# binli123/dsmil-wsi

Measured on AMD Instinct MI355X. Metric: bags/sec aggregated (10kx512), higher is better.
Workload: dtype f32; 1 GPU; DSMIL aggregator forward (FCLayer+BClassifier), c16 weights C=1, 64 bags x 10000 x 512 fp32 per GPU per pass, HBM-resident; bags_per_pass_per_gpu=64, rows=10000, feats=512, classes=1, tile_rows=128, parallelism=bag-sharded x1, streams=3, distinct_batches=3, logits_form=1, device_cus=256, persistent_grid=256

## Files before the change

dsmil-wsi_amd/csrc/agg_f2.h:

```cpp
#pragma once
#include "agg_hs.h"

namespace {

typedef _Float16 f16x8 __attribute__((ext_vector_type(8)));
typedef _Float16 f16x2 __attribute__((ext_vector_type(2)));
union F2Frag {
    unsigned u[4];
    f16x8 v;
    f32x4 f;
    f16x2 h[4];
};

constexpr int F2_BM = 64;
constexpr int F2_THREADS = 512;
constexpr int F2_MAXSTEPS = 32;
constexpr int F2_XP_F4 = F2_MAXSTEPS * 2 * 2 * F2_BM;
constexpr int F2_HP_F4 = 2 * 4 * 2 * F2_BM;
constexpr int F2_SCR = 2720;
constexpr int F2_LDS_BYTES = (F2_XP_F4 + F2_HP_F4) * 16 + F2_SCR * 4;
constexpr int F2_CHUNK_F4 = 4 * 2 * 64;
constexpr int F2_WRD = 8;
constexpr int F2_WLA = 6;
constexpr int F2_STAGGER = 0;
// ... 262 lines not shown
        const float* src = row_src(cur, sc, sinv);
        hand_over(0, true, cur, sinv);
        sQall[tid - 256] = load_q(cur);

#pragma unroll
        for (int c = 0; c < NK1; ++c) {
            ring[c][0] = *(const DSMIL_GLOBAL f32x4*)(src + 32 * c);
            ring[c][1] = *(const DSMIL_GLOBAL f32x4*)(src + 32 * c + 4);
        }
        int nitem = item + stride;
        F2Tile nxt = cur;
        bool have_next = f2_fetch(a, tiles_per_bag, n_items, stride, nitem, nxt);
        const float* nsrc = have_next ? row_src(nxt, nsc, nsinv) : src;
        __syncthreads();
        int par = 0;
        f32x4* dst0 = sXp + (long long)((o >> 1) * 4 + (o & 1)) * F2_BM + 16 * j + rr;
        while (have) {
            STAMP(0);
            const float qn = load_q(nxt);
            hand_over(par ^ 1, have_next, nxt, nsinv);
            auto refill = [&](int k) {
                if constexpr ((ABL & 2) == 0) {
                    if constexpr ((ABL & 64) != 0) {
                        ring[k][0] = __builtin_nontemporal_load((const DSMIL_GLOBAL f32x4*)(nsrc + 32 * k));
                        ring[k][1] = __builtin_nontemporal_load((const DSMIL_GLOBAL f32x4*)(nsrc + 32 * k + 4));
                    } else {
                        ring[k][0] = *(const DSMIL_GLOBAL f32x4*)(nsrc + 32 * k);
                        ring[k][1] = *(const DSMIL_GLOBAL f32x4*)(nsrc + 32 * k + 4);
                    }
                }
            };
#pragma unroll
            for (int c = 0; c < NK1; ++c) {
                if constexpr ((ABL & 16) == 0) {
                    F2Frag f[2];
                    split2h_scaled(ring[c][0], ring[c][1], sc, f);
                    f32x4* dst = dst0 + (long long)c * (8 * F2_BM);
                    dst[0] = f[0].f;
                    dst[2 * F2_BM] = f[1].f;
                }
                if constexpr ((ABL & 2) == 0) {
                    if constexpr ((ABL & 256) != 0) { if (c % 2 == 1) refill(c / 2); }
                    else if (c < NK1 / 2) refill(c);
                }
                if (c < NK1 / 2 || c % 4 == 3) __syncthreads();
                if (c == 0) STAMP(1);
                if (c == 3) STAMP(2);
                if (c == 7) STAMP(3);
                if (c == 11) STAMP(4);
                if (c == NK1 - 1) STAMP(5);
            }
            sQall[(par ^ 1) * 256 + (tid - 256)] = qn;
            int nnitem = nitem + stride;
            F2Tile nn = nxt;
            bool have_nn = false;
            float nnsc = nsc, nnsinv = nsinv;
            const float* nnsrc = nsrc;
            auto look_record = [&]() { have_nn = have_next && f2_fetch(a, tiles_per_bag, n_items, stride, nnitem, nn); };
            auto look_rows = [&]() { if (have_nn) nnsrc = row_src(nn, nnsc, nnsinv); };
            auto refill_q = [&](int q) {
                if constexpr (NK1 % 8 == 0) {
#pragma unroll
                    for (int k = NK1 / 2 + q * (NK1 / 8); k < NK1 / 2 + (q + 1) * (NK1 / 8); ++k) refill(k);
                } else if (q == 0) {
#pragma unroll
                    for (int k = NK1 / 2; k < NK1; ++k) refill(k);
                }
            };
            if (a.nonlinear) {
                refill_q(0); __syncthreads();
                refill_q(1); __syncthreads();
                look_record();
                refill_q(2); __syncthreads();
                refill_q(3); __syncthreads();
                look_rows();
            } else {
                refill_q(0); refill_q(1); refill_q(2); refill_q(3);
                look_record(); look_rows();
            }
            asm volatile("" : "+v"(nnsc), "+v"(nnsinv), "+v"(nnsrc));
            STAMP(6);
            f2_tail<ABL>(a, cur, noq, sXp, sS, sPw, sQall + par * 256, sInvAll + par * F2_BM, NKS);
            STAMP(7);
            STAMP_OUT(cur);
            item = nitem; cur = nxt; have = have_next; src = nsrc; sc = nsc;
            nitem = nnitem; nxt = nn; have_next = have_nn; nsrc = nnsrc; nsc = nnsc; nsinv = nnsinv;
            par ^= 1;
        }
        return;
    }

    const char* wbase = reinterpret_cast<const char*>(wimg + (2 * wave) * 64);
    const unsigned loff = (unsigned)lane * 16u;
    F2Frag wr[F2_WRD][2];
    auto load_w = [&](auto slot_, int s) {
        constexpr int R = decltype(slot_)::value;
        if constexpr ((ABL & 1) != 0) return;
        int sw = s < nst ? s : s - nst;
        asm volatile("" : "+s"(sw));
        const char* p = wbase + (size_t)sw * (F2_CHUNK_F4 * 16);
        wr[R][0].f = *(const DSMIL_GLOBAL f32x4*)(p + loff);
        wr[R][1].f = *(const DSMIL_GLOBAL f32x4*)(p + 1024 + loff);
    };
    auto read_x = [&](int s, F2Frag (&fb)[2][2]) {
        const f32x4* p = sXp + (long long)(s * 4 + hi) * F2_BM + l31;
#pragma unroll
        for (int g = 0; g < 2; ++g) {
            fb[g][0].f = p[32 * g];
            fb[g][1].f = p[2 * F2_BM + 32 * g];
        }
    };
    auto read_h = [&](int st, F2Frag (&fb)[2][2]) {
        const f32x4* p = sHp + (long long)((st & 3) * 2 + hi) * F2_BM + l31;
#pragma unroll
        for (int g = 0; g < 2; ++g) {
            fb[g][0].f = p[32 * g];
            fb[g][1].f = p[8 * F2_BM + 32 * g];
        }
    };
    auto mfma6 = [&](f32x16 (&acc)[2], const F2Frag (&w)[2], const F2Frag (&x)[2][2]) {
        if constexpr ((ABL & 4) != 0) {
            acc[0][0] += w[0].f[0] + w[1].f[0] + x[0][0].f[0] + x[0][1].f[0];
            acc[1][0] += x[1][0].f[0] + x[1][1].f[0];
            return;
        }
#pragma unroll
        for (int g = 0; g < 2; ++g) acc[g] = __builtin_amdgcn_mfma_f32_32x32x16_f16(w[1].v, x[g][0].v, acc[g], 0, 0, 0);
#pragma unroll
        for (int g = 0; g < 2; ++g) acc[g] = __builtin_amdgcn_mfma_f32_32x32x16_f16(w[0].v, x[g][1].v, acc[g], 0, 0, 0);
#pragma unroll
        for (int g = 0; g < 2; ++g) acc[g] = __builtin_amdgcn_mfma_f32_32x32x16_f16(w[0].v, x[g][0].v, acc[g], 0, 0, 0);
    };
    using F_ = std::false_type;
    using T_ = std::true_type;
    static_assert(F2_WRD == 8, "step groups below");
    constexpr int WLA = (ABL & 128) ? 7 : F2_WLA;
    load_w(std::integral_constant<int, 0>{}, 0);
    load_w(std::integral_constant<int, 1>{}, 1);
    load_w(std::integral_constant<int, 2>{}, 2);
    load_w(std::integral_constant<int, 3>{}, 3);
    load_w(std::integral_constant<int, 4>{}, 4);
    load_w(std::integral_constant<int, 5>{}, 5);
    if constexpr (WLA == 7) load_w(std::integral_constant<int, 6>{}, 6);
    const float ia1 = trailer[0], ia2 = trailer[1];
    __syncthreads();
    int par = 0;
    while (true) {
        const int* ctl = reinterpret_cast<const int*>(sCtl + par * 8);
        auto ctl64 = [&](int i) {
            const unsigned lo = (unsigned)__builtin_amdgcn_readfirstlane(ctl[2 * i]), hi_ = (unsigned)__builtin_amdgcn_readfirstlane(ctl[2 * i + 1]);
            return (long long)(((unsigned long long)hi_ << 32) | lo);
        };
        if (__builtin_amdgcn_readfirstlane(ctl[0]) == 0) break;
        cur.bag = (int)ctl64(1); cur.off0 = ctl64(2); cur.Nb = ctl64(3); cur.row0 = ctl64(4); cur.slot = ctl64(5);
        const float* sInv = sInvAll + par * F2_BM;
        STAMP(0);
        f32x16 Hw[2], Qw[2];
#pragma unroll
        for (int g = 0; g < 2; ++g)
#pragma unroll
            for (int r = 0; r < 16; ++r) Hw[g][r] = 0.f;
        __syncthreads();
        STAMP(1);
        F2Frag xb[2][2];
        read_x(0, xb);
#pragma unroll
        for (int s = 0; s < NKS; ++s) {
            const bool pre = s + 1 < NKS;
            if ((s & 1) && pre && f2_group_first<NK1>((s + 1) / 2)) __syncthreads();
            __builtin_amdgcn_sched_barrier(0);
            switch ((s + WLA) % 8) {
                case 0: load_w(std::integral_constant<int, 0>{}, s + WLA); break;
                case 1: load_w(std::integral_constant<int, 1>{}, s + WLA); break;
                case 2: load_w(std::integral_constant<int, 2>{}, s + WLA); break;
                case 3: load_w(std::integral_constant<int, 3>{}, s + WLA); break;
                case 4: load_w(std::integral_constant<int, 4>{}, s + WLA); break;
                case 5: load_w(std::integral_constant<int, 5>{}, s + WLA); break;
                case 6: load_w(std::integral_constant<int, 6>{}, s + WLA); break;
                default: load_w(std::integral_constant<int, 7>{}, s + WLA); break;
            }
            __builtin_amdgcn_sched_barrier(0);
            F2Frag xn[2][2];
            if (pre) read_x(s + 1, xn);
            mfma6(Hw, wr[s % 8], xb);
            if (pre) {
#pragma unroll
                for (int g = 0; g < 2; ++g)
#pragma unroll
                    for (int p = 0; p < 2; ++p) xb[g][p] = xn[g][p];
            }
            __builtin_amdgcn_sched_barrier(0);
            if (s == 7) STAMP(2);
            if (s == 15) STAMP(3);
            if (s == 23) STAMP(4);
        }
        STAMP(5);
        const float inv_sc[2] = {sInv[l31], sInv[32 + l31]};
#pragma unroll
        for (int q = 0; q < 4; ++q) {
            const f32x4 bq = *reinterpret_cast<const f32x4*>(sBias + 32 * wave + 8 * q + 4 * hi);
#pragma unroll
            for (int g = 0; g < 2; ++g) {
                const float iv = ia1 * inv_sc[g];
#pragma unroll
                for (int e = 0; e < 4; ++e) {
                    const float v = fmaf(Hw[g][4 * q + e], iv, bq[e]);
                    Hw[g][4 * q + e] = a.nonlinear ? fmaxf(v, 0.f) : v;
                }
            }
        }
        if (!a.nonlinear) {
#pragma unroll
            for (int g = 0; g < 2; ++g) Qw[g] = Hw[g];
        } else {
#pragma unroll
            for (int g = 0; g < 2; ++g) {
                float m = 0.f;
#pragma unroll
                for (int r = 0; r < 16; ++r) m = fmaxf(m, Hw[g][r]);
                m = fmaxf(m, __shfl_xor(m, 32, 64));
                if (hi == 0) sMax[wave * F2_BM + 32 * g + l31] = m;
            }
            __syncthreads();
            STAMP(6);
            float hsc[2], hinv[2];
#pragma unroll
            for (int g = 0; g < 2; ++g) {
                const int r = 32 * g + l31;
                const float m = fmaxf(fmaxf(sMax[r], sMax[F2_BM + r]), fmaxf(sMax[2 * F2_BM + r], sMax[3 * F2_BM + r]));
                hsc[g] = f2_scale(m, hinv[g]);
            }
            auto publish_h = [&]() {
#pragma unroll
                for (int g = 0; g < 2; ++g)
#pragma unroll
                    for (int sx = 0; sx < 2; ++sx) {
                        const f32x4 h0 = {Hw[g][8 * sx], Hw[g][8 * sx + 1], Hw[g][8 * sx + 2], Hw[g][8 * sx + 3]};
                        const f32x4 h1 = {Hw[g][8 * sx + 4], Hw[g][8 * sx + 5], Hw[g][8 * sx + 6], Hw[g][8 * sx + 7]};
                        F2Frag f[2];
                        split2h_scaled(h0, h1, hsc[g], f);
                        f32x4* dst = sHp + (long long)((2 * (wave & 1) + sx) * 2 + hi) * F2_BM + 32 * g + l31;
                        dst[0] = f[0].f;
                        dst[8 * F2_BM] = f[1].f;
                    }
            };
#pragma unroll
            for (int g = 0; g < 2; ++g)
#pragma unroll
                for (int r = 0; r < 16; ++r) Qw[g][r] = 0.f;
            auto step2 = [&](auto ri, auto pre_, int st) {
                constexpr int RI = decltype(ri)::value;
                constexpr bool PRE = decltype(pre_)::value;
                __builtin_amdgcn_sched_barrier(0);
                load_w(std::integral_constant<int, (RI + WLA) % F2_WRD>{}, NKS + st + WLA);
                __builtin_amdgcn_sched_barrier(0);
                F2Frag xn[2][2];
                if constexpr (PRE) read_h(st + 1, xn);
                mfma6(Qw, wr[RI], xb);
                if constexpr (PRE) {
#pragma unroll
                    for (int g = 0; g < 2; ++g)
#pragma unroll
                        for (int p = 0; p < 2; ++p) xb[g][p] = xn[g][p];
                }
                __builtin_amdgcn_sched_barrier(0);
            };
            if (wave < 2) publish_h();
            __syncthreads();
            STAMP(7);
            read_h(0, xb);
            step2(std::integral_constant<int, 0>{}, T_{}, 0);
            step2(std::integral_constant<int, 1>{}, T_{}, 1);
            step2(std::integral_constant<int, 2>{}, T_{}, 2);
            step2(std::integral_constant<int, 3>{}, F_{}, 3);
            STAMP(8);
            __syncthreads();
            if (wave >= 2) publish_h();
            __syncthreads();
            STAMP(9);
            read_h(4, xb);
            step2(std::integral_constant<int, 4>{}, T_{}, 4);
            step2(std::integral_constant<int, 5>{}, T_{}, 5);
            step2(std::integral_constant<int, 6>{}, T_{}, 6);
            step2(std::integral_constant<int, 7>{}, F_{}, 7);
#pragma unroll
            for (int q = 0; q < 4; ++q) {
                const f32x4 bq = *reinterpret_cast<const f32x4*>(sBias + QD + 32 * wave + 8 * q + 4 * hi);
#pragma unroll
                for (int g = 0; g < 2; ++g) {
                    const float iv = ia2 * hinv[g];
#pragma unroll
                    for (int e = 0; e < 4; ++e) Qw[g][4 * q + e] = fast_tanh(fmaf(Qw[g][4 * q + e], iv, bq[e]));
                }
            }
        }
        STAMP(10);
        f2_tail<ABL>(a, cur, Qw, sXp, sS, sPw, sQall + par * 256, sInv, NKS);
        STAMP(11);
        STAMP_OUT(cur);
        par ^= 1;
    }
}

__global__ __launch_bounds__(256) void k_pack_agg_f2(const float* __restrict__ q0_w, const float* __restrict__ q2_w,
                                                     _Float16* __restrict__ out, int K, int nks) {
    __shared__ float s_m[2][4];
    const int tid = threadIdx.x, lane = tid & 63, wave = tid >> 6;
    float m1 = 0.f, m2 = 0.f;
    for (long long i = tid; i < (long long)QD * K; i += 256) m1 = fmaxf(m1, fabsf(q0_w[i]));
    if (q2_w)
        for (int i = tid; i < QD * QD; i += 256) m2 = fmaxf(m2, fabsf(q2_w[i]));
    m1 = wave_max(m1);
    m2 = wave_max(m2);
    if (lane == 0) { s_m[0][wave] = m1; s_m[1][wave] = m2; }
    __syncthreads();
    m1 = fmaxf(fmaxf(s_m[0][0], s_m[0][1]), fmaxf(s_m[0][2], s_m[0][3]));
    m2 = fmaxf(fmaxf(s_m[1][0], s_m[1][1]), fmaxf(s_m[1][2], s_m[1][3]));
    float i1, i2;
    const float a1 = f2_scale(m1, i1), a2 = f2_scale(m2, i2);
    const long long per = (long long)F2_CHUNK_F4 * 8;
    const long long total = (long long)(nks + (q2_w ? 8 : 0)) * per;
    for (long long i = (long long)blockIdx.x * 256 + tid; i < total; i += (long long)gridDim.x * 256) {
        const int s = (int)(i / per);
        int r = (int)(i - s * per);
        const int e = r & 7; r >>= 3;
        const int ln = r & 63; r >>= 6;
        const int p = r & 1, t = r >> 1;
        const int l31 = ln & 31, hi = ln >> 5;
        float v;
        if (s < nks) {
            const int k = 16 * s + 8 * hi + e;
            v = k < K ? q0_w[(long long)(32 * t + l31) * K + k] * a1 : 0.f;
        } else {
            const int st = s - nks, tt = st >> 1, sx = st & 1;
            v = q2_w[(32 * t + l31) * QD + 32 * tt + 16 * sx + (e & 3) + 8 * (e >> 2) + 4 * hi] * a2;
        }
        const _Float16 h = (_Float16)v;
        out[i] = p == 0 ? h : (_Float16)(v - (float)h);
    }
    if (blockIdx.x == 0) {
        __shared__ float s_n1[4];
        float n1 = 0.f;
        for (int j = wave; j < QD; j += 4) {
            float sum = 0.f;
            for (int k = lane; k < K; k += 64) sum += fabsf(q0_w[(long long)j * K + k]);
            n1 = fmaxf(n1, wave_sum(sum));
        }
        if (lane == 0) s_n1[wave] = n1;
        __syncthreads();
        if (tid == 0) {
            float* tr = reinterpret_cast<float*>(out + (long long)(nks + 8) * per);
            tr[0] = i1;
            tr[1] = i2;
            tr[2] = fmaxf(fmaxf(s_n1[0], s_n1[1]), fmaxf(s_n1[2], s_n1[3]));
        }
    }
}

}
```

dsmil-wsi_amd/csrc/agg_f3.h:

```cpp
#pragma once
#include "agg_f2.h"

namespace {

constexpr int F3_BM = 32;
constexpr int F3_THREADS = 256;
constexpr int F3_MAX_WG = 1024;
constexpr int F3_HROW = 528;
constexpr int F3_SCR = 1600;
__host__ __device__ constexpr int f3_row_bytes(int K) { return 4 * K + 16; }
__host__ __device__ constexpr int f3_lds_bytes(int K) { return 2 * F3_BM * f3_row_bytes(K) + F3_BM * F3_HROW + F3_SCR * 4; }

__device__ __forceinline__ void f3_mfma_a(f32x16& acc, const f32x4& a_agpr, const f32x4& b) {
    asm volatile("v_mfma_f32_32x32x16_f16 %0, %1, %2, %0" : "+v"(acc) : "a"(a_agpr), "v"(b));
}
__device__ __forceinline__ void f3_mfma_a0(f32x16& acc, const f32x4& a_agpr, const f32x4& b) {
    asm volatile("v_mfma_f32_32x32x16_f16 %0, %1, %2, 0" : "=&v"(acc) : "a"(a_agpr), "v"(b));
}
__device__ __forceinline__ void f3_mfma_v(f32x16& acc, const f32x4& a, const f32x4& b) {
    asm volatile("v_mfma_f32_32x32x16_f16 %0, %1, %2, %0" : "+v"(acc) : "v"(a), "v"(b));
}
__device__ __forceinline__ void f3_mfma_v0(f32x16& acc, const f32x4& a, const f32x4& b) {
    asm volatile("v_mfma_f32_32x32x16_f16 %0, %1, %2, 0" : "=&v"(acc) : "v"(a), "v"(b));
}
#define F3_NOP() asm volatile("s_nop 15" ::: "memory")

template <int B, int E, class F>
__device__ __forceinline__ void f3_static_for(F&& f) {
    if constexpr (B < E) {
        f(std::integral_constant<int, B>{});
        f3_static_for<B + 1, E>(f);
    }
}

struct F3Work {
    int bag;
    long long off0, Nb, row0;
};

struct F3Cur {
    int item, b, tile;
};
__device__ __forceinline__ F3Cur f3_next(F3Cur c, int tiles_per_bag) {
    ++c.item;
    if (++c.tile == tiles_per_bag) { c.tile = 0; ++c.b; }
    return c;
}

__device__ __forceinline__ bool f3_fetch(const AttendArgs& a, int tiles_per_bag, int end, F3Cur& c, F3Work& w, const F3Work* hint = nullptr) {
    const __attribute__((address_space(4))) long long* offs = (const __attribute__((address_space(4))) long long*)(uintptr_t)a.offsets;
    while (c.item < end) {
        const int bag = a.bag0 + c.b;
        long long off0, Nb;
        if (hint && hint->bag == bag) { off0 = hint->off0; Nb = hint->Nb; }
        else { off0 = offs[bag]; Nb = offs[bag + 1] - off0; }
        const long long row0 = (long long)c.tile * F3_BM;
        if (row0 < Nb) {
            w.bag = bag; w.off0 = off0; w.Nb = Nb; w.row0 = row0;
            return true;
        }
        if (tiles_per_bag) c.item += tiles_per_bag - c.tile;
        c.tile = 0;
        ++c.b;
    }
    return false;
}

template <int NK1, bool TWO, int DBG = 0>
__global__ __launch_bounds__(F3_THREADS, 1) void k_attend_f3(AttendArgs a, const float* __restrict__ rowmax, int tiles_per_bag,
                                                             int n_items, int per_wg) {
    static_assert(NK1 % 4 == 0 && NK1 >= 4 && NK1 <= 16, "K a multiple of 128 up to 512");
    constexpr int K = 32 * NK1, NKS = 2 * NK1, NG = NK1 / 2;
    constexpr int RB = f3_row_bytes(K), BUF = F3_BM * RB;
    constexpr int NC = TWO ? 2 : 1;
    constexpr bool W2_STREAM = NK1 > 8;
    constexpr int NMOVE = 2;
    extern __shared__ __attribute__((aligned(16))) float smem[];
    char* sX = reinterpret_cast<char*>(smem);
    char* sH = sX + 2 * BUF;
    float* scr = reinterpret_cast<float*>(sH + F3_BM * F3_HROW);
    float* sS = scr;
    float* sBias = scr + 768;
    float* sPall = scr + 1024;
    float* sInvAll = scr + 1280;
    float* sQ = scr + 1344;
    const int tid = threadIdx.x, lane = tid & 63;
    const int wave = __builtin_amdgcn_readfirstlane(tid >> 6);
    const int l31 = lane & 31, hi = lane >> 5;
    const f32x4* wimg = reinterpret_cast<const f32x4*>(a.wpk);
    const float* trailer = reinterpret_cast<const float*>(wimg + (long long)(NKS + 8) * F2_CHUNK_F4);
    const float* feats = reinterpret_cast<const float*>(a.feats);
    const float scale = 0.08838834764831845f;

    F3Cur pos;
    pos.item = (int)blockIdx.x * per_wg;
    if (a.tile_pre) {
        const int real = ((const __attribute__((address_space(4))) int*)(uintptr_t)a.tile_pre)[a.n_bags];
        n_items = n_items < real ? n_items : real;
        if (pos.item >= n_items) return;
        pos.b = tile_owner(a.tile_pre, a.n_bags, pos.item);
        pos.tile = pos.item - a.tile_pre[pos.b];
    } else {
        pos.b = pos.item / tiles_per_bag;
        pos.tile = pos.item - pos.b * tiles_per_bag;
    }
    const int item_end = pos.item + per_wg < n_items ? pos.item + per_wg : n_items;
    F3Work cur, nxt, nn;
    if (!f3_fetch(a, tiles_per_bag, item_end, pos, cur)) return;

    F2Frag w1[NKS][2], w2[8][2];
#pragma unroll
    for (int s = 0; s < NKS; ++s)
#pragma unroll
        for (int p = 0; p < 2; ++p) w1[s][p].f = wimg[(long long)s * F2_CHUNK_F4 + (2 * wave + p) * 64 + lane];
    const f32x4* w2p1 = wimg + (long long)NKS * F2_CHUNK_F4 + (2 * wave + 1) * 64 + lane;
#pragma unroll
    for (int st = 0; st < 8; ++st) {
        w2[st][0].f = wimg[(long long)(NKS + st) * F2_CHUNK_F4 + (2 * wave) * 64 + lane];
        if constexpr (!W2_STREAM) w2[st][1].f = w2p1[(long long)st * F2_CHUNK_F4];
    }
    const float ia1 = trailer[0], ia2 = trailer[1];
    const float hb_n1 = trailer[2] * 16384.f;
    const float hb_b = wave_max(fmaxf(fabsf(a.q0_b[lane]), fabsf(a.q0_b[lane + 64])));
    sBias[tid] = tid < QD ? a.q0_b[tid] : a.q2_b[tid - QD];
#pragma unroll
    for (int s = 0; s < NKS; ++s)
#pragma unroll
        for (int p = 0; p < 2; ++p) asm volatile("" : "+a"(w1[s][p].f));

    const int rr = lane & 7, o = lane >> 3;
    const int myrow = 8 * wave + rr;
    f32x4 ring[NG][2];
    auto row_raw = [&](const F3Work& w, float& rm, long long& phys, long long& logical) {
        long long gr = w.row0 + myrow;
        if (gr >= w.Nb) gr = w.Nb - 1;
        rm = rowmax[w.off0 + gr];
        const long long* mp = a.rowmap ? reinterpret_cast<const long long*>(a.rowmap) + (w.off0 + gr) : reinterpret_cast<const long long*>(a.offsets);
        phys = *mp;
        logical = w.off0 + gr;
    };
    auto row_done = [&](float rm, long long phys, long long logical, float& sc, float& sinv) -> const float* {
        sc = f2_scale(rm, sinv);
        return feats + (a.rowmap ? phys : logical) * (long long)K + 8 * o;
    };
    auto row_src = [&](const F3Work& w, float& sc, float& sinv) -> const float* {
        float rm;
        long long phys, logical;
        row_raw(w, rm, phys, logical);
        asm volatile("" : "+v"(phys));
        return row_done(rm, phys, logical, sc, sinv);
    };
    auto fill = [&](const float* src, int c) {
        ring[c][0] = *(const DSMIL_GLOBAL f32x4*)(src + 64 * c);
        ring[c][1] = *(const DSMIL_GLOBAL f32x4*)(src + 64 * c + 4);
    };
    char* const cut_dst = sX + myrow * RB + 16 * o;
    auto cut_write = [&](int pb, int c, float sc) {
        F2Frag f[2];
        split2h_scaled(ring[c][0], ring[c][1], sc, f);
        char* d = cut_dst + pb * BUF + 128 * c;
        *reinterpret_cast<f32x4*>(d) = f[0].f;
        *reinterpret_cast<f32x4*>(d + 2 * K) = f[1].f;
    };

    F2Frag cutf[2];
    auto cut_piece = [&](int pb, auto s_c, auto j_c, float sc, const float* refill_src) {
        constexpr int s_ = decltype(s_c)::value, j = decltype(j_c)::value;
        constexpr int c = s_ / 4, ph = (s_ % 4) * 3 + j;
        if constexpr (c < NG) {
            char* d = cut_dst + pb * BUF + 128 * c;
            if constexpr (ph < 8) {
                constexpr int i = ph / 2;
                const float va = i < 2 ? ring[c][0][(2 * i) & 3] : ring[c][1][(2 * i) & 3];
                const float vb = i < 2 ? ring[c][0][(2 * i + 1) & 3] : ring[c][1][(2 * i + 1) & 3];
                if constexpr (ph % 2 == 0) {
                    unsigned h;
                    asm("v_fma_mixlo_f16 %0, %1, %3, 0\n\tv_fma_mixhi_f16 %0, %2, %3, 0" : "=&v"(h) : "v"(va), "v"(vb), "v"(sc));
                    cutf[0].u[i] = h;
                } else {
                    unsigned l;
                    const unsigned h = cutf[0].u[i];
                    asm("v_fma_mixlo_f16 %0, %1, %3, -%4 op_sel_hi:[0,0,1]\n\tv_fma_mixhi_f16 %0, %2, %3, -%4 op_sel:[0,0,1] op_sel_hi:[0,0,1]"
                        : "=&v"(l) : "v"(va), "v"(vb), "v"(sc), "v"(h));
                    cutf[1].u[i] = l;
                }
            } else if constexpr (ph == 8) {
                *reinterpret_cast<f32x4*>(d) = cutf[0].f;
            } else if constexpr (ph == 9) {
                *reinterpret_cast<f32x4*>(d + 2 * K) = cutf[1].f;
            } else if constexpr (ph == 10) {
                if constexpr (DBG != 4 && c < NG - NMOVE) fill(refill_src, c);
            }
        }
    };

    float sc_c = 1.f, sinv_c = 1.f, sc_n = 1.f, sinv_n = 1.f, sc_nn = 1.f, sinv_nn = 1.f;
    const float* src_c = row_src(cur, sc_c, sinv_c);
#pragma unroll
    for (int c = 0; c < NG; ++c) fill(src_c, c);
    F3Cur pos_n = f3_next(pos, tiles_per_bag);
    bool has_next = f3_fetch(a, tiles_per_bag, item_end, pos_n, nxt);
    const float* src_n = has_next ? row_src(nxt, sc_n, sinv_n) : src_c;
    if (!has_next) { nxt = cur; sc_n = sc_c; sinv_n = sinv_c; }
#pragma unroll
    for (int c = 0; c < NG; ++c) {
        cut_write(0, c, sc_c);
        fill(src_n, c);
    }
    if (o == 0) sInvAll[myrow] = sinv_c;
    F3Cur pos_nn = f3_next(pos_n, tiles_per_bag);
    bool has_nn = has_next && f3_fetch(a, tiles_per_bag, item_end, pos_nn, nn);
    const float* src_nn = has_nn ? row_src(nn, sc_nn, sinv_nn) : src_n;
    if (!has_nn) { nn = nxt; sc_nn = sc_n; sinv_nn = sinv_n; }

    float bacc[NC][8];
    float l_run[NC];
    float m_bag[NC];
    auto reset_acc = [&]() {
#pragma unroll
        for (int c = 0; c < NC; ++c) {
            l_run[c] = 0.f;
#pragma unroll
            for (int e = 0; e < 8; ++e) bacc[c][e] = 0.f;
        }
    };
    reset_acc();
#pragma unroll
    for (int c = 0; c < NC; ++c) m_bag[c] = 0.f;
    int qbag = -1;
    float* sPw = sPall + wave * 64;

    unsigned long long stamps[16];
#pragma unroll
    for (int i = 0; i < 16; ++i) stamps[i] = 0;
    auto STAMP = [&](int i) {
        if constexpr (DBG >= 1) {
            __builtin_amdgcn_sched_barrier(0);
            asm volatile("s_waitcnt vmcnt(63) lgkmcnt(0)" ::: "memory");
            stamps[i] = __builtin_readcyclecounter();
            __builtin_amdgcn_sched_barrier(0);
        }
    };
    for (int t = 0;; ++t) {
        const int buf = t & 1;
        STAMP(0);
        if (cur.bag != qbag) {
            __syncthreads();
            if (tid < NC * QD) sQ[tid] = a.qmax[(long long)cur.bag * a.C * QD + tid];
            qbag = cur.bag;
            __syncthreads();
#pragma unroll
            for (int c = 0; c < NC; ++c) m_bag[c] = wave_sum(fabsf(sQ[c * QD + lane]) + fabsf(sQ[c * QD + 64 + lane])) * scale;
        }
        F3Cur pos_n3 = f3_next(pos_nn, tiles_per_bag);
        F3Work n3 = nn;
        float rm_n3;
        long long phys_n3, log_n3;
        const bool has_n3 = has_nn && f3_fetch(a, tiles_per_bag, item_end, pos_n3, n3, &nn);
        if (!has_n3) n3 = nn;
        row_raw(n3, rm_n3, phys_n3, log_n3);
        __syncthreads();
        STAMP(1);
        const char* xb_ = sX + buf * BUF + l31 * RB + 16 * hi;
        const float* sInv = sInvAll + buf * F3_BM;
        f32x16 Hacc[2];
        {
            F2Frag xs[3][2];
            auto rd = [&](int s_, F2Frag (&d)[2]) {
                d[0].f = *reinterpret_cast<const f32x4*>(xb_ + 32 * s_);
                d[1].f = *reinterpret_cast<const f32x4*>(xb_ + 2 * K + 32 * s_);
            };
            rd(0, xs[0]);
            rd(1, xs[1]);
            f3_static_for<0, NKS>([&](auto s_c) {
                constexpr int s = decltype(s_c)::value;
                using J0 = std::integral_constant<int, 0>;
                using J1 = std::integral_constant<int, 1>;
                using J2 = std::integral_constant<int, 2>;
                if constexpr (DBG != 3 && DBG != 5 && s + 2 < NKS) rd(s + 2, xs[(s + 2) % 3]);
                __builtin_amdgcn_sched_barrier(0);
                if constexpr (s == 0) f3_mfma_a0(Hacc[0], w1[s][1].f, xs[s % 3][0].f);
                else f3_mfma_a(Hacc[s & 1], w1[s][1].f, xs[s % 3][0].f);
                if constexpr (DBG != 2 && DBG != 5) cut_piece(buf ^ 1, s_c, J0{}, sc_n, src_nn);
                __builtin_amdgcn_sched_barrier(0);
                if constexpr (s == 0) f3_mfma_a0(Hacc[1], w1[s][0].f, xs[s % 3][1].f);
                else f3_mfma_a(Hacc[~s & 1], w1[s][0].f, xs[s % 3][1].f);
                if constexpr (DBG != 2 && DBG != 5) cut_piece(buf ^ 1, s_c, J1{}, sc_n, src_nn);
                __builtin_amdgcn_sched_barrier(0);
                f3_mfma_a(Hacc[s & 1], w1[s][0].f, xs[s % 3][0].f);
                if constexpr (DBG != 2 && DBG != 5) cut_piece(buf ^ 1, s_c, J2{}, sc_n, src_nn);
                __builtin_amdgcn_sched_barrier(0);
                if constexpr (s == 7) STAMP(10);
                if constexpr (s == 15) STAMP(11);
                if constexpr (s == 23) STAMP(12);
            });
            F3_NOP();
        }
        if (o == 0) sInvAll[(buf ^ 1) * F3_BM + myrow] = sinv_n;
        if constexpr (W2_STREAM) {
#pragma unroll
            for (int st = 0; st < 8; ++st) w2[st][1].f = *(const DSMIL_GLOBAL f32x4*)(w2p1 + (long long)st * F2_CHUNK_F4);
        }
        STAMP(2);
        const float rinv1 = sInv[l31];
        const float iv1 = ia1 * rinv1;
        f32x16 H;
#pragma unroll
        for (int q = 0; q < 4; ++q) {
            const f32x4 bq = *reinterpret_cast<const f32x4*>(sBias + 32 * wave + 8 * q + 4 * hi);
#pragma unroll
            for (int e = 0; e < 4; ++e) H[4 * q + e] = fmaxf(fmaf(Hacc[0][4 * q + e] + Hacc[1][4 * q + e], iv1, bq[e]), 0.f);
        }
        STAMP(3);
        float hsc, hinv;
        hsc = f2_scale(fmaf(hb_n1, rinv1, hb_b), hinv);
#pragma unroll
        for (int sx = 0; sx < 2; ++sx) {
            const f32x4 h0 = {H[8 * sx], H[8 * sx + 1], H[8 * sx + 2], H[8 * sx + 3]};
            const f32x4 h1 = {H[8 * sx + 4], H[8 * sx + 5], H[8 * sx + 6], H[8 * sx + 7]};
            F2Frag f[2];
            split2h_scaled(h0, h1, hsc, f);
            char* d = sH + l31 * F3_HROW + ((2 * wave + sx) * 2 + hi) * 16;
            *reinterpret_cast<f32x4*>(d) = f[0].f;
            *reinterpret_cast<f32x4*>(d + 256) = f[1].f;
        }
        __syncthreads();
        STAMP(4);
        f32x16 Qacc[2];
        {
            const char* hb_ = sH + l31 * F3_HROW + 16 * hi;
            F2Frag hs[3][2];
            auto rdh = [&](int st_, F2Frag (&d)[2]) {
                d[0].f = *reinterpret_cast<const f32x4*>(hb_ + 32 * st_);
                d[1].f = *reinterpret_cast<const f32x4*>(hb_ + 256 + 32 * st_);
            };
            rdh(0, hs[0]);
            rdh(1, hs[1]);
#pragma unroll
            for (int st = 0; st < 8; ++st) {
                if (st + 2 < 8) rdh(st + 2, hs[(st + 2) % 3]);
                __builtin_amdgcn_sched_barrier(0);
                if (st == 0) {
                    f3_mfma_v0(Qacc[0], w2[st][1].f, hs[st % 3][0].f);
                    f3_mfma_v0(Qacc[1], w2[st][0].f, hs[st % 3][1].f);
                } else {
                    f3_mfma_v(Qacc[st & 1], w2[st][1].f, hs[st % 3][0].f);
                    f3_mfma_v(Qacc[~st & 1], w2[st][0].f, hs[st % 3][1].f);
                }
                f3_mfma_v(Qacc[st & 1], w2[st][0].f, hs[st % 3][0].f);
                if (DBG != 4 && st < NMOVE) fill(src_nn, NG - NMOVE + st);
                __builtin_amdgcn_sched_barrier(0);
            }
            F3_NOP();
        }
        STAMP(5);
        {
            const float iv2 = ia2 * hinv;
            float s0 = 0.f, s1 = 0.f;
#pragma unroll
            for (int q = 0; q < 4; ++q) {
                const f32x4 bq = *reinterpret_cast<const f32x4*>(sBias + QD + 32 * wave + 8 * q + 4 * hi);
                const f32x4 u0 = *reinterpret_cast<const f32x4*>(sQ + 32 * wave + 8 * q + 4 * hi);
                f32x4 u1 = u0;
                if constexpr (TWO) u1 = *reinterpret_cast<const f32x4*>(sQ + QD + 32 * wave + 8 * q + 4 * hi);
#pragma unroll
                for (int e = 0; e < 4; ++e) {
                    const float qv = fast_tanh(fmaf(Qacc[0][4 * q + e] + Qacc[1][4 * q + e], iv2, bq[e]));
                    s0 = fmaf(qv, u0[e], s0);
                    if constexpr (TWO) s1 = fmaf(qv, u1[e], s1);
                }
            }
            sS[((wave * 2 + hi) * 2 + 0) * F3_BM + l31] = s0;
            if constexpr (TWO) sS[((wave * 2 + hi) * 2 + 1) * F3_BM + l31] = s1;
        }
        STAMP(6);
        __syncthreads();
        STAMP(7);
        {
            const long long grow = cur.row0 + l31;
            const bool valid = grow < cur.Nb;
            const float rinv = sInv[l31];
#pragma unroll
            for (int c = 0; c < NC; ++c) {
                auto part = [&](int i) { return sS[(i * 2 + c) * F3_BM + l31]; };
                const float s = (((part(0) + part(1)) + (part(2) + part(3))) + ((part(4) + part(5)) + (part(6) + part(7)))) * scale;
                const float p = valid ? expf(s - m_bag[c]) : 0.f;
                if (hi == 0) l_run[c] += p;
                if (DBG == 0 && wave == 0 && hi == 0 && valid) a.scores[(cur.off0 + grow) * (long long)a.C + c] = s;
                if (hi == 0) sPw[c * F3_BM + l31] = p * rinv;
            }
        }
        STAMP(8);
        if (lane < K / 8) {
            const char* xv = sX + buf * BUF + (8 * wave) * RB + 16 * lane;
#pragma unroll
            for (int j = 0; j < 8; ++j) {
                F2Frag f0, f1;
                f0.f = *reinterpret_cast<const f32x4*>(xv + j * RB);
                f1.f = *reinterpret_cast<const f32x4*>(xv + j * RB + 2 * K);
#pragma unroll
                for (int c = 0; c < NC; ++c) {
                    const float w = sPw[c * F3_BM + 8 * wave + j];
#pragma unroll
                    for (int e = 0; e < 8; ++e) {
                        bacc[c][e] = fmaf((float)f0.v[e], w, bacc[c][e]);
                        bacc[c][e] = fmaf((float)f1.v[e], w, bacc[c][e]);
                    }
                }
            }
        }
        STAMP(9);
        if constexpr (DBG >= 1) {
            if (tid == 0 && !TWO && cur.row0 + F3_BM <= cur.Nb) {
                unsigned long long* so = reinterpret_cast<unsigned long long*>(a.scores + (cur.off0 + cur.row0));
#pragma unroll
                for (int i = 0; i < 16; ++i) so[i] = stamps[i];
            }
        }
        if (!has_next || nxt.bag != cur.bag) {
            const long long slot = (long long)blockIdx.x + cur.bag;
            float* red = reinterpret_cast<float*>(sH);
            __syncthreads();
            if (lane < K / 8) {
#pragma unroll
                for (int c = 0; c < NC; ++c) {
                    float* d = red + (wave * NC + c) * K + 8 * lane;
                    *reinterpret_cast<f32x4*>(d) = f32x4{bacc[c][0], bacc[c][1], bacc[c][2], bacc[c][3]};
                    *reinterpret_cast<f32x4*>(d + 4) = f32x4{bacc[c][4], bacc[c][5], bacc[c][6], bacc[c][7]};
                }
            }
            __syncthreads();
            for (int i = tid; i < NC * K; i += F3_THREADS) {
                const int c = i / K, k = i - c * K;
                const float v = (red[(0 * NC + c) * K + k] + red[(1 * NC + c) * K + k]) + (red[(2 * NC + c) * K + k] + red[(3 * NC + c) * K + k]);
                a.part_B[(slot * a.C + c) * (long long)a.Kv + k] = v;
            }
            if (wave == 0) {
#pragma unroll
                for (int c = 0; c < NC; ++c) {
                    const float lsum = wave_sum(hi == 0 ? l_run[c] : 0.f);
                    if (lane == 0) {
                        float* ml = a.part_ml + (slot * a.C + c) * 2;
                        ml[0] = m_bag[c];
                        ml[1] = lsum;
                    }
                }
            }
            reset_acc();
        }
        STAMP(13);
        if constexpr (DBG >= 1) {
            if (tid == 0 && !TWO && cur.row0 + F3_BM <= cur.Nb)
                reinterpret_cast<unsigned long long*>(a.scores + (cur.off0 + cur.row0))[13] = stamps[13];
        }
        if (!has_next) break;
        cur = nxt; nxt = nn; nn = n3;
        has_next = has_nn; has_nn = has_n3;
        pos_nn = pos_n3;
        sc_c = sc_n; sinv_c = sinv_n;
        sc_n = sc_nn; sinv_n = sinv_nn; src_n = src_nn;
        asm volatile("" : "+v"(rm_n3), "+v"(phys_n3));
        src_nn = row_done(rm_n3, phys_n3, log_n3, sc_nn, sinv_nn);
    }
}

}
```

Measured before the change: 108,100 bags/s.

## Switch attend kernel MFMA from 32x32x16 to 16x16x32 tiles

Replaces the 32x32x16 f16 MFMA with 16x16x32 in both the FC and Q GEMMs of the attend kernel. It remaps the weight-fragment indexing, the X/H shared-memory reads, the epilogue and the score reduction to the new tile shape, and enlarges scratch space for 16 partial sums per row. The aim is shorter MFMA dependency chains and finer interleaving with the next-tile cut and fill work. The cost is more MFMA instructions and LDS reads, plus the risk of a mismatch with the existing weight packing layout.

After: 111,400 bags/s, median of 6. 3.0% higher.

```diff
diff --git a/dsmil-wsi_amd/csrc/agg_f2.h b/dsmil-wsi_amd/csrc/agg_f2.h
--- a/dsmil-wsi_amd/csrc/agg_f2.h
+++ b/dsmil-wsi_amd/csrc/agg_f2.h
@@ -588,6 +588,20 @@
     }
 }
 
+struct F3UnitK {
+    int unit, k;
+};
+__host__ __device__ constexpr int f3_unit(int ub, int m) { return 32 * (ub >> 1) + 16 * (m >> 3) + 8 * (ub & 1) + (m & 7); }
+__host__ __device__ constexpr F3UnitK f3_frag_map(int nk1, int chunk, int ub, int lane, int e) {
+    const int m = lane & 15, g = lane >> 4;
+    if (chunk < nk1) return {f3_unit(ub, m), 32 * chunk + 8 * g + e};
+    return {f3_unit(ub, m), 32 * (chunk - nk1) + 16 * (g >> 1) + 4 * (g & 1) + (e & 3) + 8 * (e >> 2)};
+}
+__host__ __device__ constexpr long long f3_frag_slot(int chunk, int ub, int plane, int lane) {
+    const int m = lane & 15, g = lane >> 4;
+    return (long long)(2 * chunk + (g >> 1)) * F2_CHUNK_F4 + ((ub >> 1) * 2 + plane) * 64 + 32 * (g & 1) + (f3_unit(ub, m) & 31);
+}
+
 __global__ __launch_bounds__(256) void k_pack_agg_f2(const float* __restrict__ q0_w, const float* __restrict__ q2_w,
                                                      _Float16* __restrict__ out, int K, int nks) {
     __shared__ float s_m[2][4];
diff --git a/dsmil-wsi_amd/csrc/agg_f3.h b/dsmil-wsi_amd/csrc/agg_f3.h
--- a/dsmil-wsi_amd/csrc/agg_f3.h
+++ b/dsmil-wsi_amd/csrc/agg_f3.h
@@ -7,21 +7,21 @@
 constexpr int F3_THREADS = 256;
 constexpr int F3_MAX_WG = 1024;
 constexpr int F3_HROW = 528;
-constexpr int F3_SCR = 1600;
+constexpr int F3_SCR = 1856;
 __host__ __device__ constexpr int f3_row_bytes(int K) { return 4 * K + 16; }
 __host__ __device__ constexpr int f3_lds_bytes(int K) { return 2 * F3_BM * f3_row_bytes(K) + F3_BM * F3_HROW + F3_SCR * 4; }
 
-__device__ __forceinline__ void f3_mfma_a(f32x16& acc, const f32x4& a_agpr, const f32x4& b) {
-    asm volatile("v_mfma_f32_32x32x16_f16 %0, %1, %2, %0" : "+v"(acc) : "a"(a_agpr), "v"(b));
-}
-__device__ __forceinline__ void f3_mfma_a0(f32x16& acc, const f32x4& a_agpr, const f32x4& b) {
-    asm volatile("v_mfma_f32_32x32x16_f16 %0, %1, %2, 0" : "=&v"(acc) : "a"(a_agpr), "v"(b));
-}
-__device__ __forceinline__ void f3_mfma_v(f32x16& acc, const f32x4& a, const f32x4& b) {
-    asm volatile("v_mfma_f32_32x32x16_f16 %0, %1, %2, %0" : "+v"(acc) : "v"(a), "v"(b));
-}
-__device__ __forceinline__ void f3_mfma_v0(f32x16& acc, const f32x4& a, const f32x4& b) {
-    asm volatile("v_mfma_f32_32x32x16_f16 %0, %1, %2, 0" : "=&v"(acc) : "v"(a), "v"(b));
+__device__ __forceinline__ void f3_mfma_a(f32x4& acc, const f32x4& a_agpr, const f32x4& b) {
+    asm volatile("v_mfma_f32_16x16x32_f16 %0, %1, %2, %0" : "+v"(acc) : "a"(a_agpr), "v"(b));
+}
+__device__ __forceinline__ void f3_mfma_a0(f32x4& acc, const f32x4& a_agpr, const f32x4& b) {
+    asm volatile("v_mfma_f32_16x16x32_f16 %0, %1, %2, 0" : "=&v"(acc) : "a"(a_agpr), "v"(b));
+}
+__device__ __forceinline__ void f3_mfma_v(f32x4& acc, const f32x4& a, const f32x4& b) {
+    asm volatile("v_mfma_f32_16x16x32_f16 %0, %1, %2, %0" : "+v"(acc) : "v"(a), "v"(b));
+}
+__device__ __forceinline__ void f3_mfma_v0(f32x4& acc, const f32x4& a, const f32x4& b) {
+    asm volatile("v_mfma_f32_16x16x32_f16 %0, %1, %2, 0" : "=&v"(acc) : "v"(a), "v"(b));
 }
 #define F3_NOP() asm volatile("s_nop 15" ::: "memory")
 
@@ -80,13 +80,15 @@
     char* sH = sX + 2 * BUF;
     float* scr = reinterpret_cast<float*>(sH + F3_BM * F3_HROW);
     float* sS = scr;
-    float* sBias = scr + 768;
-    float* sPall = scr + 1024;
-    float* sInvAll = scr + 1280;
-    float* sQ = scr + 1344;
+    float* sBias = scr + 1024;
+    float* sPall = scr + 1280;
+    float* sInvAll = scr + 1536;
+    float* sQ = scr + 1600;
     const int tid = threadIdx.x, lane = tid & 63;
     const int wave = __builtin_amdgcn_readfirstlane(tid >> 6);
     const int l31 = lane & 31, hi = lane >> 5;
+    const int l15 = lane & 15, g = lane >> 4;
+    const int ubase = 32 * wave + 16 * (g >> 1) + 4 * (g & 1);
     const f32x4* wimg = reinterpret_cast<const f32x4*>(a.wpk);
     const float* trailer = reinterpret_cast<const float*>(wimg + (long long)(NKS + 8) * F2_CHUNK_F4);
     const float* feats = reinterpret_cast<const float*>(a.feats);
@@ -108,25 +110,31 @@
     F3Work cur, nxt, nn;
     if (!f3_fetch(a, tiles_per_bag, item_end, pos, cur)) return;
 
-    F2Frag w1[NKS][2], w2[8][2];
-#pragma unroll
-    for (int s = 0; s < NKS; ++s)
-#pragma unroll
-        for (int p = 0; p < 2; ++p) w1[s][p].f = wimg[(long long)s * F2_CHUNK_F4 + (2 * wave + p) * 64 + lane];
-    const f32x4* w2p1 = wimg + (long long)NKS * F2_CHUNK_F4 + (2 * wave + 1) * 64 + lane;
-#pragma unroll
-    for (int st = 0; st < 8; ++st) {
-        w2[st][0].f = wimg[(long long)(NKS + st) * F2_CHUNK_F4 + (2 * wave) * 64 + lane];
-        if constexpr (!W2_STREAM) w2[st][1].f = w2p1[(long long)st * F2_CHUNK_F4];
-    }
+    F2Frag w1[NK1][2][2], w2[4][2][2];
+#pragma unroll
+    for (int s = 0; s < NK1; ++s)
+#pragma unroll
+        for (int uh = 0; uh < 2; ++uh)
+#pragma unroll
+            for (int p = 0; p < 2; ++p) w1[s][uh][p].f = wimg[f3_frag_slot(s, 2 * wave + uh, p, lane)];
+    const f32x4* w2p1 = wimg + f3_frag_slot(NK1, 2 * wave, 1, lane);
+#pragma unroll
+    for (int st = 0; st < 4; ++st)
+#pragma unroll
+        for (int uh = 0; uh < 2; ++uh) {
+            w2[st][uh][0].f = wimg[f3_frag_slot(NK1 + st, 2 * wave + uh, 0, lane)];
+            if constexpr (!W2_STREAM) w2[st][uh][1].f = w2p1[(long long)2 * st * F2_CHUNK_F4 + 8 * uh];
+        }
     const float ia1 = trailer[0], ia2 = trailer[1];
     const float hb_n1 = trailer[2] * 16384.f;
     const float hb_b = wave_max(fmaxf(fabsf(a.q0_b[lane]), fabsf(a.q0_b[lane + 64])));
     sBias[tid] = tid < QD ? a.q0_b[tid] : a.q2_b[tid - QD];
 #pragma unroll
-    for (int s = 0; s < NKS; ++s)
-#pragma unroll
-        for (int p = 0; p < 2; ++p) asm volatile("" : "+a"(w1[s][p].f));
+    for (int s = 0; s < NK1; ++s)
+#pragma unroll
+        for (int uh = 0; uh < 2; ++uh)
+#pragma unroll
+            for (int p = 0; p < 2; ++p) asm volatile("" : "+a"(w1[s][uh][p].f));
 
     const int rr = lane & 7, o = lane >> 3;
     const int myrow = 8 * wave + rr;
@@ -166,7 +174,7 @@
     F2Frag cutf[2];
     auto cut_piece = [&](int pb, auto s_c, auto j_c, float sc, const float* refill_src) {
         constexpr int s_ = decltype(s_c)::value, j = decltype(j_c)::value;
-        constexpr int c = s_ / 4, ph = (s_ % 4) * 3 + j;
+        constexpr int c = s_ / 2, ph = (s_ % 2) * 8 + j;
         if constexpr (c < NG) {
             char* d = cut_dst + pb * BUF + 128 * c;
             if constexpr (ph < 8) {
@@ -261,117 +269,122 @@
         row_raw(n3, rm_n3, phys_n3, log_n3);
         __syncthreads();
         STAMP(1);
-        const char* xb_ = sX + buf * BUF + l31 * RB + 16 * hi;
+        const char* xb_ = sX + buf * BUF + (2 * l15) * RB + 16 * g;
         const float* sInv = sInvAll + buf * F3_BM;
-        f32x16 Hacc[2];
+        f32x4 Hacc[2][2];
         {
-            F2Frag xs[3][2];
-            auto rd = [&](int s_, F2Frag (&d)[2]) {
-                d[0].f = *reinterpret_cast<const f32x4*>(xb_ + 32 * s_);
-                d[1].f = *reinterpret_cast<const f32x4*>(xb_ + 2 * K + 32 * s_);
+            F2Frag xs[2][2][2];
+            auto rd = [&](int s_, int rh, int p, F2Frag& d) {
+                d.f = *reinterpret_cast<const f32x4*>(xb_ + rh * RB + p * (2 * K) + 64 * s_);
             };
-            rd(0, xs[0]);
-            rd(1, xs[1]);
-            f3_static_for<0, NKS>([&](auto s_c) {
+#pragma unroll
+            for (int q = 0; q < 4; ++q) rd(0, q >> 1, q & 1, xs[0][q >> 1][q & 1]);
+            f3_static_for<0, NK1>([&](auto s_c) {
                 constexpr int s = decltype(s_c)::value;
-                using J0 = std::integral_constant<int, 0>;
-                using J1 = std::integral_constant<int, 1>;
-                using J2 = std::integral_constant<int, 2>;
-                if constexpr (DBG != 3 && DBG != 5 && s + 2 < NKS) rd(s + 2, xs[(s + 2) % 3]);
+                f3_static_for<0, 12>([&](auto j_c) {
+                    constexpr int j = decltype(j_c)::value;
+                    constexpr int pr = j / 4, uh = (j >> 1) & 1, rh = j & 1;
+                    constexpr int pa = pr == 0 ? 1 : 0, pb = pr == 1 ? 1 : 0;
+                    __builtin_amdgcn_sched_barrier(0);
+                    if constexpr (s == 0 && pr == 0) f3_mfma_a0(Hacc[uh][rh], w1[s][uh][pa].f, xs[s % 2][rh][pb].f);
+                    else f3_mfma_a(Hacc[uh][rh], w1[s][uh][pa].f, xs[s % 2][rh][pb].f);
+                    if constexpr (j < 4) {
+                        if constexpr (DBG != 3 && DBG != 5 && s + 1 < NK1) rd(s + 1, j >> 1, j & 1, xs[(s + 1) % 2][j >> 1][j & 1]);
+                    } else if constexpr (DBG != 2 && DBG != 5) {
+                        cut_piece(buf ^ 1, s_c, std::integral_constant<int, j - 4>{}, sc_n, src_nn);
+                    }
+                });
                 __builtin_amdgcn_sched_barrier(0);
-                if constexpr (s == 0) f3_mfma_a0(Hacc[0], w1[s][1].f, xs[s % 3][0].f);
-                else f3_mfma_a(Hacc[s & 1], w1[s][1].f, xs[s % 3][0].f);
-                if constexpr (DBG != 2 && DBG != 5) cut_piece(buf ^ 1, s_c, J0{}, sc_n, src_nn);
-                __builtin_amdgcn_sched_barrier(0);
-                if constexpr (s == 0) f3_mfma_a0(Hacc[1], w1[s][0].f, xs[s % 3][1].f);
-                else f3_mfma_a(Hacc[~s & 1], w1[s][0].f, xs[s % 3][1].f);
-                if constexpr (DBG != 2 && DBG != 5) cut_piece(buf ^ 1, s_c, J1{}, sc_n, src_nn);
-                __builtin_amdgcn_sched_barrier(0);
-                f3_mfma_a(Hacc[s & 1], w1[s][0].f, xs[s % 3][0].f);
-                if constexpr (DBG != 2 && DBG != 5) cut_piece(buf ^ 1, s_c, J2{}, sc_n, src_nn);
-                __builtin_amdgcn_sched_barrier(0);
-                if constexpr (s == 7) STAMP(10);
-                if constexpr (s == 15) STAMP(11);
-                if constexpr (s == 23) STAMP(12);
+                if constexpr (s == 3) STAMP(10);
+                if constexpr (s == 7) STAMP(11);
+                if constexpr (s == 11) STAMP(12);
             });
             F3_NOP();
         }
         if (o == 0) sInvAll[(buf ^ 1) * F3_BM + myrow] = sinv_n;
         if constexpr (W2_STREAM) {
 #pragma unroll
-            for (int st = 0; st < 8; ++st) w2[st][1].f = *(const DSMIL_GLOBAL f32x4*)(w2p1 + (long long)st * F2_CHUNK_F4);
+            for (int st = 0; st < 4; ++st)
+#pragma unroll
+                for (int uh = 0; uh < 2; ++uh) w2[st][uh][1].f = *(const DSMIL_GLOBAL f32x4*)(w2p1 + (long long)2 * st * F2_CHUNK_F4 + 8 * uh);
         }
         STAMP(2);
-        const float rinv1 = sInv[l31];
-        const float iv1 = ia1 * rinv1;
-        f32x16 H;
-#pragma unroll
-        for (int q = 0; q < 4; ++q) {
-            const f32x4 bq = *reinterpret_cast<const f32x4*>(sBias + 32 * wave + 8 * q + 4 * hi);
-#pragma unroll
-            for (int e = 0; e < 4; ++e) H[4 * q + e] = fmaxf(fmaf(Hacc[0][4 * q + e] + Hacc[1][4 * q + e], iv1, bq[e]), 0.f);
+        const float rinv1[2] = {sInv[2 * l15], sInv[2 * l15 + 1]};
+#pragma unroll
+        for (int uh = 0; uh < 2; ++uh) {
+            const f32x4 bq = *reinterpret_cast<const f32x4*>(sBias + ubase + 8 * uh);
+#pragma unroll
+            for (int rh = 0; rh < 2; ++rh) {
+                const float iv1 = ia1 * rinv1[rh];
+#pragma unroll
+                for (int e = 0; e < 4; ++e) Hacc[uh][rh][e] = fmaxf(fmaf(Hacc[uh][rh][e], iv1, bq[e]), 0.f);
+            }
         }
         STAMP(3);
-        float hsc, hinv;
-        hsc = f2_scale(fmaf(hb_n1, rinv1, hb_b), hinv);
-#pragma unroll
-        for (int sx = 0; sx < 2; ++sx) {
-            const f32x4 h0 = {H[8 * sx], H[8 * sx + 1], H[8 * sx + 2], H[8 * sx + 3]};
-            const f32x4 h1 = {H[8 * sx + 4], H[8 * sx + 5], H[8 * sx + 6], H[8 * sx + 7]};
+        float hinv[2];
+#pragma unroll
+        for (int rh = 0; rh < 2; ++rh) {
+            const float hsc = f2_scale(fmaf(hb_n1, rinv1[rh], hb_b), hinv[rh]);
             F2Frag f[2];
-            split2h_scaled(h0, h1, hsc, f);
-            char* d = sH + l31 * F3_HROW + ((2 * wave + sx) * 2 + hi) * 16;
+            split2h_scaled(Hacc[0][rh], Hacc[1][rh], hsc, f);
+            char* d = sH + (2 * l15 + rh) * F3_HROW + 64 * wave + 16 * g;
             *reinterpret_cast<f32x4*>(d) = f[0].f;
             *reinterpret_cast<f32x4*>(d + 256) = f[1].f;
         }
         __syncthreads();
         STAMP(4);
-        f32x16 Qacc[2];
+        f32x4 Qacc[2][2];
         {
-            const char* hb_ = sH + l31 * F3_HROW + 16 * hi;
-            F2Frag hs[3][2];
-            auto rdh = [&](int st_, F2Frag (&d)[2]) {
-                d[0].f = *reinterpret_cast<const f32x4*>(hb_ + 32 * st_);
-                d[1].f = *reinterpret_cast<const f32x4*>(hb_ + 256 + 32 * st_);
+            const char* hb_ = sH + (2 * l15) * F3_HROW + 16 * g;
+            F2Frag hs[2][2][2];
+            auto rdh = [&](int st_, F2Frag (&d)[2][2]) {
+#pragma unroll
+                for (int rh = 0; rh < 2; ++rh)
+#pragma unroll
+                    for (int p = 0; p < 2; ++p) d[rh][p].f = *reinterpret_cast<const f32x4*>(hb_ + rh * F3_HROW + 256 * p + 64 * st_);
             };
             rdh(0, hs[0]);
-            rdh(1, hs[1]);
-#pragma unroll
-            for (int st = 0; st < 8; ++st) {
-                if (st + 2 < 8) rdh(st + 2, hs[(st + 2) % 3]);
+            f3_static_for<0, 4>([&](auto st_c) {
+                constexpr int st = decltype(st_c)::value;
+                if constexpr (st + 1 < 4) rdh(st + 1, hs[(st + 1) % 2]);
+                f3_static_for<0, 12>([&](auto j_c) {
+                    constexpr int j = decltype(j_c)::value;
+                    constexpr int pr = j / 4, uh = (j >> 1) & 1, rh = j & 1;
+                    constexpr int pa = pr == 0 ? 1 : 0, pb = pr == 1 ? 1 : 0;
+                    __builtin_amdgcn_sched_barrier(0);
+                    if constexpr (st == 0 && pr == 0) f3_mfma_v0(Qacc[uh][rh], w2[st][uh][pa].f, hs[st % 2][rh][pb].f);
+                    else f3_mfma_v(Qacc[uh][rh], w2[st][uh][pa].f, hs[st % 2][rh][pb].f);
+                    if constexpr (DBG != 4 && st == 0 && j % 6 == 5 && j / 6 < NMOVE) fill(src_nn, NG - NMOVE + j / 6);
+                });
                 __builtin_amdgcn_sched_barrier(0);
-                if (st == 0) {
-                    f3_mfma_v0(Qacc[0], w2[st][1].f, hs[st % 3][0].f);
-                    f3_mfma_v0(Qacc[1], w2[st][0].f, hs[st % 3][1].f);
-                } else {
-                    f3_mfma_v(Qacc[st & 1], w2[st][1].f, hs[st % 3][0].f);
-                    f3_mfma_v(Qacc[~st & 1], w2[st][0].f, hs[st % 3][1].f);
-                }
-                f3_mfma_v(Qacc[st & 1], w2[st][0].f, hs[st % 3][0].f);
-                if (DBG != 4 && st < NMOVE) fill(src_nn, NG - NMOVE + st);
-                __builtin_amdgcn_sched_barrier(0);
-            }
+            });
             F3_NOP();
         }
         STAMP(5);
         {
-            const float iv2 = ia2 * hinv;
-            float s0 = 0.f, s1 = 0.f;
-#pragma unroll
-            for (int q = 0; q < 4; ++q) {
-                const f32x4 bq = *reinterpret_cast<const f32x4*>(sBias + QD + 32 * wave + 8 * q + 4 * hi);
-                const f32x4 u0 = *reinterpret_cast<const f32x4*>(sQ + 32 * wave + 8 * q + 4 * hi);
+            float s0[2] = {0.f, 0.f}, s1[2] = {0.f, 0.f};
+#pragma unroll
+            for (int uh = 0; uh < 2; ++uh) {
+                const f32x4 bq = *reinterpret_cast<const f32x4*>(sBias + QD + ubase + 8 * uh);
+                const f32x4 u0 = *reinterpret_cast<const f32x4*>(sQ + ubase + 8 * uh);
                 f32x4 u1 = u0;
-                if constexpr (TWO) u1 = *reinterpret_cast<const f32x4*>(sQ + QD + 32 * wave + 8 * q + 4 * hi);
-#pragma unroll
-                for (int e = 0; e < 4; ++e) {
-                    const float qv = fast_tanh(fmaf(Qacc[0][4 * q + e] + Qacc[1][4 * q + e], iv2, bq[e]));
-                    s0 = fmaf(qv, u0[e], s0);
-                    if constexpr (TWO) s1 = fmaf(qv, u1[e], s1);
+                if constexpr (TWO) u1 = *reinterpret_cast<const f32x4*>(sQ + QD + ubase + 8 * uh);
+#pragma unroll
+                for (int rh = 0; rh < 2; ++rh) {
+                    const float iv2 = ia2 * hinv[rh];
+#pragma unroll
+                    for (int e = 0; e < 4; ++e) {
+                        const float qv = fast_tanh(fmaf(Qacc[uh][rh][e], iv2, bq[e]));
+                        s0[rh] = fmaf(qv, u0[e], s0[rh]);
+                        if constexpr (TWO) s1[rh] = fmaf(qv, u1[e], s1[rh]);
+                    }
                 }
             }
-            sS[((wave * 2 + hi) * 2 + 0) * F3_BM + l31] = s0;
-            if constexpr (TWO) sS[((wave * 2 + hi) * 2 + 1) * F3_BM + l31] = s1;
+#pragma unroll
+            for (int rh = 0; rh < 2; ++rh) {
+                sS[((wave * 4 + g) * 2 + 0) * F3_BM + 2 * l15 + rh] = s0[rh];
+                if constexpr (TWO) sS[((wave * 4 + g) * 2 + 1) * F3_BM + 2 * l15 + rh] = s1[rh];
+            }
         }
         STAMP(6);
         __syncthreads();
@@ -383,7 +396,8 @@
 #pragma unroll
             for (int c = 0; c < NC; ++c) {
                 auto part = [&](int i) { return sS[(i * 2 + c) * F3_BM + l31]; };
-                const float s = (((part(0) + part(1)) + (part(2) + part(3))) + ((part(4) + part(5)) + (part(6) + part(7)))) * scale;
+                auto quad = [&](int i) { return (part(i) + part(i + 1)) + (part(i + 2) + part(i + 3)); };
+                const float s = ((quad(0) + quad(4)) + (quad(8) + quad(12))) * scale;
                 const float p = valid ? expf(s - m_bag[c]) : 0.f;
                 if (hi == 0) l_run[c] += p;
                 if (DBG == 0 && wave == 0 && hi == 0 && valid) a.scores[(cur.off0 + grow) * (long long)a.C + c] = s;
```
